# pansanity666/TransHuman

Measured on AMD Instinct MI355X. Metric: rays/sec (512x512, 64 samples/ray), higher is better.
Workload: dtype f32 (fp16 hi/lo x3 MFMA emulation)

## Files before the change

include/transhuman_hip.h:

```cpp
#ifndef TRANSHUMAN_HIP_H
#define TRANSHUMAN_HIP_H

#include <stddef.h>
#include <stdint.h>

#ifdef __cplusplus
extern "C" {
#endif

#define TH_ABI_VERSION 12

typedef struct th_ctx th_ctx;
typedef void* th_stream;

int         th_abi_version(void);
const char* th_last_error(void);
int         th_ctx_create(int device, th_ctx** out);
void        th_ctx_destroy(th_ctx* ctx);
size_t      th_sizeof(const char* type_name);

enum { TH_PROF_HULL = 0, TH_PROF_DPARF = 1, TH_PROF_GATHER = 2, TH_PROF_MLP = 3, TH_PROF_COMPOSITE = 4,
       TH_PROF_VIT = 5, TH_PROF_FOLD = 6 , TH_PROF_PHASES = 8 };
int th_profile_enable(th_ctx* ctx, int on);
int th_profile_read(th_ctx* ctx, double* ms_out, int64_t* count_out);
int th_host_wait_read(th_ctx* ctx, double* ms_out);
int th_clock_probe(th_ctx* ctx, int64_t* out_dev , th_stream stream);
int th_fused_cycles(th_ctx* ctx, int64_t* counters_dev);

typedef struct {
    const float* w;
    const float* b;
    int out_f;
    int in_f;
} th_linear;

typedef struct {
    th_linear fc_0, alpha_res_0;
    th_linear key0, val0;
    th_linear key1, val1;
    th_linear fc_1, fc_2, fc_3, alpha_fc;
    th_linear feature_fc, rgb_res_0, view_fc, rgb_res_1, fc_4, rgb_fc;
    th_linear upsample_color;
} th_mlp_weights;

typedef struct {
    const float *ln1_w, *ln1_b, *ln2_w, *ln2_b;
    th_linear qkv, proj, fc1, fc2;
} th_vit_block;

int th_set_mlp_weights(th_ctx* ctx, const th_mlp_weights* w, th_stream stream);
int th_set_mlp_mode(th_ctx* ctx, int mode);
int th_set_fused_waves(th_ctx* ctx, int waves);
int th_set_tok_gather(th_ctx* ctx, int on);
int th_set_tex_rows(th_ctx* ctx, int on);

#define TH_RANGE_SLOTS 8
#define TH_RANGE_FP16_LIMIT 0x7B53u
#define TH_RANGE_FP16_FLOOR 0x2400u
int th_set_vit_mode(th_ctx* ctx, int mode);
int th_range_snapshot(th_ctx* ctx, th_stream stream);
// ... 257 lines not shown
```

transhuman_amd/csrc/k_mlp_fused8_kernel.h:

```cpp
#pragma once
#include "k_mlp_fused_kernel.h"

typedef float f8_f4 __attribute__((ext_vector_type(4)));
typedef short f8_s4 __attribute__((ext_vector_type(4)));
typedef short f8_s8 __attribute__((ext_vector_type(8)));

#define F8_THREADS 512
#define F8_PART_FLOATS (3 * 8 * 32)
#define F8_PSTR 12
#define F8_MISC_FLOATS (F8_PSTR * 32 + F8_PART_FLOATS + 32 + 8)
#define F8_LDS_BYTES (ABUF_BYTES + MBUF_BYTES + F8_MISC_FLOATS * 4)
static_assert(F8_LDS_BYTES <= 163840, "the 8-wave tile must fit the CU's LDS");

#define F8_MFMA(A, B, C) __builtin_amdgcn_mfma_f32_16x16x32_f16((A), (B), (C), 0, 0, 0)

template <int CT>
__device__ __forceinline__ void f8_load_w(const uint4* __restrict__ wl, int t, uint4 (&w)[CT][2]) {
    const uint4* p = wl + (long long)t * (CT * 2 * 64);
#pragma unroll
    for (int c = 0; c < CT; ++c) {
        w[c][0] = p[(c * 2 + 0) * 64];
        w[c][1] = p[(c * 2 + 1) * 64];
    }
}
#define F8_WSLICE(L, wave, ct) ((L).w + (long long)(wave) * (L).KB * ((ct) * 2 * 64))

template <int NR, int ROWSTEP, bool PERM>
__device__ __forceinline__ void f8_load_x(const char* __restrict__ ahi, const char* __restrict__ alo, int aoff, int t,
                                          h8 (&xh)[NR], h8 (&xl)[NR]) {
    const int ko = (PERM ? 32 : 64) * t;
#pragma unroll
    for (int r = 0; r < NR; ++r) {
        xh[r] = *reinterpret_cast<const h8*>(ahi + r * ROWSTEP + aoff + ko);
        xl[r] = *reinterpret_cast<const h8*>(alo + r * ROWSTEP + aoff + ko);
    }
}
template <bool PERM>
__device__ __forceinline__ int f8_aoff(int lane, int str) {
    const int l = lane & 15, g = lane >> 4;
    return PERM ? l * str + 16 * (g >> 1) + 256 * (g & 1) : l * str + 16 * g;
}

template <int CT, int RT, int NR, int R0, bool FIRST>
__device__ __forceinline__ void f8_mfma_half(const uint4 (&w)[CT][2], const h8 (&xh)[NR], const h8 (&xl)[NR], f8_f4 (&acc)[CT][RT]) {
    const f8_f4 zero = {0.f, 0.f, 0.f, 0.f};
// ... 130 lines not shown
__device__ __forceinline__ void f8_mfma_dual(const uint4 (&r3)[2][2], const uint4 (&ra)[1][2], const h8 (&mh)[1], const h8 (&ml)[1],
                                             const h8 (&xh)[NV], const h8 (&xl)[NV], f8_f4 (&a3)[2][2], f8_f4 (&va)[1][RT]) {
    const f8_f4 zero = {0.f, 0.f, 0.f, 0.f};
#pragma unroll
    for (int t = 0; t < 3; ++t) {
        const int wp = t == 0 ? 1 : 0;
        const bool lo = t == 1;
        const bool first = FIRST && t == 0;
        a3[0][H] = F8_MFMA(*reinterpret_cast<const h8*>(&r3[0][wp]), lo ? ml[0] : mh[0], first ? zero : a3[0][H]);
#pragma unroll
        for (int r = 0; r < NV; ++r) {
            va[0][R0 + r] = F8_MFMA(*reinterpret_cast<const h8*>(&ra[0][wp]), lo ? xl[r] : xh[r], first ? zero : va[0][R0 + r]);
            if (r == 0) a3[1][H] = F8_MFMA(*reinterpret_cast<const h8*>(&r3[1][wp]), lo ? ml[0] : mh[0], first ? zero : a3[1][H]);
        }
    }
}

template <int V>
__global__ __launch_bounds__(F8_THREADS, 2) void mlp_fused8_kernel(FusedParams P_arg) {
#define PK P_arg
    struct F8Dbg { long long* dbg; };
    const F8Dbg P{PK.dbg};
    extern __shared__ __attribute__((aligned(16))) char lds[];
    char* abuf = lds;
    char* mbuf = lds + ABUF_BYTES;
    float* misc = reinterpret_cast<float*>(lds + ABUF_BYTES + MBUF_BYTES);
    float* probs = misc;
    float* part = misc + F8_PSTR * 32;
    float* sig = part + F8_PART_FLOATS;
    int* flag = reinterpret_cast<int*>(sig + 32);

    const int tid = threadIdx.x, lane = tid & 63, wave = tid >> 6;
    const int l15 = lane & 15, g4 = lane >> 4;
    const int tile = (int)((blockIdx.x & 7) * (gridDim.x >> 3) + (blockIdx.x >> 3));
    const int pbase = tile * FM_PTS;
    if (pbase >= PK.P) return;
    const int npts = min(FM_PTS, PK.P - pbase);
    const int fm_dbg_tile = tile;
    const int zoff = 0;
    constexpr int ROWS = 32 * V, RT = 2 * V;
    constexpr int RS256 = 16 * STR256;
    int dbg_i = 1;
    long long dbg_t = 0;
    long long* dbg_keep = reinterpret_cast<long long*>(flag + 2);
    constexpr float inv_v = 1.0f / (float)V;
    unsigned rmax = 0u;
    unsigned seen_s = 0u, seen_p = 0u, seen_n = 0u, seen_i = 0u, seen_4 = 0u;
    char* a256_lo = abuf + ROWS * STR256;

    struct TexPre { unsigned h0, h1; fm_u4 rq; };
    auto tex_fetch = [&]() __attribute__((always_inline)) {
        int tl = tile;
        asm volatile("" : "+s"(tl));
        TexPre t;
        const unsigned* hb = PK.tex_hdr + (long long)tl * 512;
        t.h0 = hb[lane];
        t.h1 = hb[64 + lane];
        t.rq = (fm_u4){0u, 0u, 0u, 0u};
        if (tid < 64 * V) t.rq = *reinterpret_cast<const fm_u4*>(PK.tex_rec + (long long)tl * V * 32 * 8 + tid * 4);
        return t;
    };
    auto fill_tex = [&](const TexPre& pre, auto rgb, auto&& under) __attribute__((always_inline)) {
        constexpr bool RGB = decltype(rgb)::value;
        constexpr int TSTR = 1040, TMAX = 103, NK = (TMAX + 7) / 8, NR = 4 * V;
        static_assert(TMAX * TSTR <= ABUF_BYTES, "a pass of texel rows must fit the operand buffer");
        int wv = __builtin_amdgcn_readfirstlane(wave), tl = tile;
        asm volatile("" : "+s"(wv), "+s"(tl));
        const unsigned* hb = PK.tex_hdr + (long long)tl * 512;
        unsigned h0 = pre.h0, h1 = pre.h1;
        const int npass = __builtin_amdgcn_readfirstlane((int)(h0 >> 16));
        char* recl = reinterpret_cast<char*>(misc);
        static_assert(32 * V * 32 <= (F8_PSTR * 32 + F8_PART_FLOATS) * 4, "row records must fit probs + part");
        unsigned fv[NR][4] = {};
        f32x2 bias_lo = {0.f, 0.f}, bias_hi = {0.f, 0.f};
        if constexpr (!RGB) {
            const float4 b4 = *reinterpret_cast<const float4*>(PK.ar0.bias + 4 * lane);
            bias_lo = (f32x2){b4.x, b4.y};
            bias_hi = (f32x2){b4.z, b4.w};
        }
        for (int p = 0; p < npass; ++p) {
            if (p > 0) {
                FM_SYNCL();
                h0 = hb[p * 128 + lane];
                h1 = hb[p * 128 + 64 + lane];
            }
            const int U = __builtin_amdgcn_readfirstlane((int)(h0 & 0xffffu));
            {
                constexpr int NA = 7, NB = 10;
                const char* mbase = reinterpret_cast<const char*>(RGB ? PK.tex_map2 : PK.tex_map);
                const unsigned loff = (unsigned)lane * 16u;
                const int last = U - 1;
                fm_u4 ta[NA], tb[NB - NA], tc[NK - NB];
#pragma unroll
                for (int k = 0; k < NA; ++k) {
                    const int i = min(wv + 8 * k, last);
                    const unsigned id = (unsigned)__builtin_amdgcn_readlane((int)h0, 8 + i);
                    ta[k] = *reinterpret_cast<const fm_u4*>(mbase + TX_ADDR(id));
                }
                const bool more = U > 8 * NA, most = U > 8 * NB;
                if (more) {
#pragma unroll
                    for (int k = NA; k < NB; ++k) {
                        const int i = min(wv + 8 * k, last);
                        const unsigned id = (unsigned)__builtin_amdgcn_readlane((int)h1, i - 56);
                        tb[k - NA] = *reinterpret_cast<const fm_u4*>(mbase + TX_ADDR(id));
                    }
                }
                if (most) {
#pragma unroll
                    for (int k = NB; k < NK; ++k) {
                        const int i = min(wv + 8 * k, last);
                        const unsigned id = (unsigned)__builtin_amdgcn_readlane((int)h1, i - 56);
                        tc[k - NB] = *reinterpret_cast<const fm_u4*>(mbase + TX_ADDR(id));
                    }
                }
                if (p == 0) {
                    under();
                    if (tid < 64 * V) *reinterpret_cast<fm_u4*>(recl + tid * 16) = pre.rq;
                }
                int wv2 = wv;
                asm volatile("" : "+s"(wv2));
#pragma unroll
                for (int k = 0; k < NA; ++k) *reinterpret_cast<fm_u4*>(abuf + min(wv2 + 8 * k, last) * TSTR + lane * 16) = ta[k];
                if (more) {
#pragma unroll
                    for (int k = NA; k < NB; ++k) *reinterpret_cast<fm_u4*>(abuf + min(wv2 + 8 * k, last) * TSTR + lane * 16) = tb[k - NA];
                }
                if (most) {
#pragma unroll
                    for (int k = NB; k < NK; ++k) *reinterpret_cast<fm_u4*>(abuf + min(wv2 + 8 * k, last) * TSTR + lane * 16) = tc[k - NB];
                }
            }
            FM_SYNCL();
            const int sh2 = npass == 1 ? 2 : npass == 2 ? 1 : 0;
            const int cofs = lane * 16;
            struct RowIn { float4 a, b, c, d; fm_u4 q0; };
            auto issue = [&](int k, const fm_u4& o, RowIn& r) __attribute__((always_inline)) {
                r.q0 = *reinterpret_cast<const fm_u4*>(recl + (wv + 8 * k) * 32);
                r.a = *reinterpret_cast<const float4*>(abuf + (o[0] + cofs));
                r.b = *reinterpret_cast<const float4*>(abuf + (o[1] + cofs));
                r.c = *reinterpret_cast<const float4*>(abuf + (o[2] + cofs));
                r.d = *reinterpret_cast<const float4*>(abuf + (o[3] + cofs));
            };
            auto offs = [&](int k) __attribute__((always_inline)) {
                return *reinterpret_cast<const fm_u4*>(recl + (wv + 8 * k) * 32 + 16);
            };
            auto blend = [&](int k, const RowIn& r, auto sel) __attribute__((always_inline)) {
// ... 15 lines not shown
                    n2 = __builtin_bit_cast(unsigned, h0f); n3 = __builtin_bit_cast(unsigned, h1f);
                } else {
                    lo = __builtin_elementwise_max(lo + bias_lo, (f32x2){0.f, 0.f});
                    hi = __builtin_elementwise_max(hi + bias_hi, (f32x2){0.f, 0.f});
                    split_pair(lo[0], lo[1], n0, n2);
                    split_pair(hi[0], hi[1], n1, n3);
                }
                if constexpr (decltype(sel)::value) {
                    const bool mine = ((k & 3) >> sh2) == p;
                    fv[k][0] = mine ? n0 : fv[k][0]; fv[k][1] = mine ? n1 : fv[k][1];
                    fv[k][2] = mine ? n2 : fv[k][2]; fv[k][3] = mine ? n3 : fv[k][3];
                } else {
                    fv[k][0] = n0; fv[k][1] = n1; fv[k][2] = n2; fv[k][3] = n3;
                }
            };
            auto rows_loop = [&](auto sel) __attribute__((always_inline)) {
                RowIn in[2];
                fm_u4 of[2];
                of[0] = offs(0);
                of[1] = offs(1);
                issue(0, of[0], in[0]);
#pragma unroll
                for (int k = 0; k < NR; ++k) {
                    if (k + 1 < NR) issue(k + 1, of[(k + 1) & 1], in[(k + 1) & 1]);
                    if (k + 2 < NR) of[k & 1] = offs(k + 2);
                    FM_SB();
                    blend(k, in[k & 1], sel);
                    FM_SB();
                }
            };
            if (npass == 1) rows_loop(std::false_type{});
            else rows_loop(std::true_type{});
        }
        FM_SYNCL();
        if constexpr (RGB) {
#pragma unroll
            for (int k = 0; k < NR; ++k)
                *reinterpret_cast<fm_u4*>(abuf + (wv + 8 * k) * TSTR + lane * 16) = (fm_u4){fv[k][0], fv[k][1], fv[k][2], fv[k][3]};
        } else {
#pragma unroll
            for (int k = 0; k < NR; ++k) {
                range_acc<true>(rmax, fv[k][0]);
                range_acc<true>(rmax, fv[k][1]);
                *reinterpret_cast<uint2*>(abuf + (wv + 8 * k) * STR256 + lane * 8) = make_uint2(fv[k][0], fv[k][1]);
                *reinterpret_cast<uint2*>(a256_lo + (wv + 8 * k) * STR256 + lane * 8) = make_uint2(fv[k][2], fv[k][3]);
            }
            range_commit(PK.range, TH_RANGE_P, seen_p, rmax);
        }
    };

    if (PK.dbg != nullptr && tid == 0 && (tile & 15) == 0) {
        atomicAdd(reinterpret_cast<unsigned long long*>(PK.dbg), 1ull);
        dbg_t = clock64();
        dbg_keep[0] = dbg_t;
        dbg_keep[1] = wall_clock64();
    }
    fm_u4 rv4 = {0u, 0u, 0u, 0u};
    unsigned rv1 = 0u;
    static_assert(TH_RANGE_S == 1 && TH_RANGE_P == 2 && TH_RANGE_N == 3 && TH_RANGE_INTER == 4 && TH_RANGE_F4 == 5, "range slots 1..5");
    if (PK.range != nullptr) {
        const unsigned* rtab = PK.range + zoff;
        rv4 = (fm_u4){rtab[1], rtab[2], rtab[3], rtab[4]};
        rv1 = rtab[5];
    }
    TexPre tex_pre = tex_fetch(), tex_pre2;

    int vsel[2] = {0, 0};
    float vdv[2] = {0.f, 0.f};
    f8_f4 acc2[2][RT];
    {
        constexpr int STOK_STR = 1040;
        static_assert(32 * V * STOK_STR <= ABUF_BYTES, "T' rows must fit the operand buffer");
        char* pe_hi = mbuf;
        char* pe_lo = mbuf + 32 * STR64;
        const int pt = tid & 255, prow = pt >> 3, pc = pt & 7, ppl = tid >> 8;
        const int psrc = min(prow, npts - 1);
        const uint4 pe_v = *reinterpret_cast<const uint4*>(PK.pe + (long long)(pbase + psrc) * 128 + 64 * ppl + 8 * pc);
        char* wsp_hi = mbuf + 16384;
        char* wsp_lo = wsp_hi + 32 * STRVD;
        const unsigned* hdr = reinterpret_cast<const unsigned*>(PK.stok) + (long long)((PK.P + 31) / 32 * 32) * 16 + (long long)tile * 128;
        const unsigned h0 = hdr[lane], h1 = hdr[64 + lane];
        const int ns = tid / 7, nk = tid - 7 * ns;
        int slot = -1;
        float nw = 0.f;
        if (tid < 224) {
            const unsigned* rec = reinterpret_cast<const unsigned*>(PK.stok) + (long long)(pbase + min(ns, npts - 1)) * 16;
            slot = (int)rec[nk];
            nw = __builtin_bit_cast(float, rec[8 + nk]);
        }
        const unsigned zq = 0u;
        const float inv_t = PK.t_inv[zoff];
        uint4 wq[2][2][2];
        const uint4* wl = F8_WSLICE(PK.w16.fc_0pe, wave, 2) + lane;
        f8_load_w<2>(wl, 0, wq[0]);
        f8_load_w<2>(wl, 1, wq[1]);
        const float4 b0[2] = {f8_bias(PK.fc_0pe.bias, wave * 32, lane), f8_bias(PK.fc_0pe.bias, wave * 32 + 16, lane)};
        if (tid < 2 * 32 * STRVD / 16) reinterpret_cast<uint4*>(wsp_hi)[tid] = make_uint4(zq, zq, zq, zq);
        *reinterpret_cast<uint4*>((ppl ? pe_lo : pe_hi) + prow * STR64 + 16 * pc) = pe_v;
        const int U = __builtin_amdgcn_readfirstlane((int)h0);
        FM_SB();
        auto slot_centre = [&](int u) {
            const int d = (2 + u) >> 1;
            const unsigned src = d < 64 ? (unsigned)__builtin_amdgcn_readlane((int)h0, d) : (unsigned)__builtin_amdgcn_readlane((int)h1, d - 64);
            return (int)((src >> (16 * ((2 + u) & 1))) & 0xffffu);
        };
#pragma unroll
        for (int c = 0; c < 2; ++c)
#pragma unroll
            for (int r = 0; r < RT; ++r) acc2[c][r] = (f8_f4){0.f, 0.f, 0.f, 0.f};
        f8_f4 a1[2][2] = {{{0.f, 0.f, 0.f, 0.f}, {0.f, 0.f, 0.f, 0.f}}, {{0.f, 0.f, 0.f, 0.f}, {0.f, 0.f, 0.f, 0.f}}};
        const int wv = __builtin_amdgcn_readfirstlane(wave);
        const int aoffw = f8_aoff<false>(lane, STRVD), aoffp = f8_aoff<false>(lane, STR64);
        for (int u0 = 0; u0 < U; u0 += 32) {
            const int nU = min(32, U - u0);
            if (u0 > 0) {
                FM_SYNCL();
                if (tid < 2 * 32 * STRVD / 16) reinterpret_cast<uint4*>(wsp_hi)[tid] = make_uint4(zq, zq, zq, zq);
            }
            for (int u = wv; u < nU; u += 8) {
                const int cu = slot_centre(u0 + u);
                const char* g = reinterpret_cast<const char*>(PK.tsplit) + (long long)cu * 1024 + lane * 16;
#pragma unroll
                for (int vw = 0; vw < V; ++vw)
                    __builtin_amdgcn_global_load_lds((fm_gptr)(g + (long long)vw * PK.t_nc * 1024),
                                                     (fm_lptr)(abuf + (vw * 32 + u) * STOK_STR), 16, 0, 0);
            }
            FM_SYNCL();
            if (slot >= u0 && slot < u0 + 32) {
                _Float16 hi, lo;
                split_h(nw, hi, lo);
                *reinterpret_cast<_Float16*>(wsp_hi + ns * STRVD + 2 * (slot - u0)) = hi;
                *reinterpret_cast<_Float16*>(wsp_lo + ns * STRVD + 2 * (slot - u0)) = lo;
            }
            if (u0 == 0) {
#pragma unroll
                for (int t = 0; t < 2; ++t) {
                    h8 xh[2], xl[2];
                    f8_load_x<2, 16 * STR64, false>(pe_hi, pe_lo, aoffp, t, xh, xl);
                    if (t == 0) f8_mfma_half<2, 2, 2, 0, true>(wq[0], xh, xl, a1);
                    else f8_mfma_half<2, 2, 2, 0, false>(wq[1], xh, xl, a1);
                }
            }
            FM_SYNC();
            {
                h8 xh[2], xl[2];
                f8_load_x<2, 16 * STRVD, false>(wsp_hi, wsp_lo, aoffw, 0, xh, xl);
                const int tq = l15 >> 2, tc = 8 * (l15 & 3);
                const int ro0 = min(8 * g4 + tq, nU - 1) * STOK_STR + tc, ro1 = min(8 * g4 + 4 + tq, nU - 1) * STOK_STR + tc;
                typedef __attribute__((address_space(3))) f8_s4* f8_lp;
#pragma unroll
                for (int r = 0; r < V; ++r)
#pragma unroll
                    for (int c = 0; c < 2; ++c) {
                        const char* rb = abuf + r * 32 * STOK_STR + 2 * (wave * 32 + c * 16);
                        const f8_s4 h0 = __builtin_amdgcn_ds_read_tr16_b64_v4i16((f8_lp)(rb + ro0));
                        const f8_s4 h1 = __builtin_amdgcn_ds_read_tr16_b64_v4i16((f8_lp)(rb + ro1));
                        const f8_s4 l0 = __builtin_amdgcn_ds_read_tr16_b64_v4i16((f8_lp)(rb + ro0 + 512));
// ... 186 lines not shown
    f8_gemm_rt<RT, 2, RS256, true, true>(abuf, a256_lo, STR256, F8_WSLICE(PK.w16.fc_2, wave, 2), 8, lane, acc2, wk2);
    const float4 bi[2] = {f8_bias(PK.fc_2.bias, wave * 32, lane), f8_bias(PK.fc_2.bias, wave * 32 + 16, lane)};
#pragma unroll
    for (int q = 0; q < 2; ++q) {
        const int i = tid + F8_THREADS * q, row = i >> 5, c = i & 31;
        float x = 0.f;
        if (PK.rgb_all != 2 && c < 27 && row < npts) {
            const long long vr = PK.vd_sel ? (long long)(vsel[q] / PK.vd_div) : (long long)(pbase + row);
            x = PK.vd[vr * 27 + c];
        }
        vdv[q] = x;
    }
    FM_SYNCL();
#pragma unroll
    for (int c = 0; c < 2; ++c) {
#pragma unroll
        for (int r = 0; r < RT; ++r) acc2[c][r] = f8_finish(acc2[c][r], bi[c], PK.fc_2.inv_scale, true);
#pragma unroll
        for (int h = 0; h < 2; ++h) {
            f8_f4 m = acc2[c][h];
#pragma unroll
            for (int r = 1; r < V; ++r) m = m + acc2[c][2 * r + h];
            m = m * (f8_f4){inv_v, inv_v, inv_v, inv_v};
            f8_store_h<STR256>(m, h * 16 + l15, wave * 32 + c * 16, mbuf, mbuf + 32 * STR256, lane, rmax);
        }
#pragma unroll
        for (int r = 0; r < RT; ++r) f8_store_h<STR256>(acc2[c][r], r * 16 + l15, wave * 32 + c * 16, abuf, a256_lo, lane, rmax);
    }
    range_commit(PK.range, TH_RANGE_INTER, seen_i, rmax);
    FM_SYNCL();

    char* vd_hi = mbuf + MBUF_VD_OFF;
    char* vd_lo = vd_hi + 32 * STRVD;
    tex_pre2 = tex_fetch();
    f8_f4 va[1][RT];
    {
        f8_f4 a3[2][2];
        const float4 aw[2] = {f8_bias(PK.alpha_w, wave * 32, lane), f8_bias(PK.alpha_w, wave * 32 + 16, lane)};
        const float4 b3[2] = {f8_bias(PK.fc_3.bias, wave * 32, lane), f8_bias(PK.fc_3.bias, wave * 32 + 16, lane)};
        if (PK.rgb_all != 2) {
            constexpr int T = 8;
            const uint4* w3l = F8_WSLICE(PK.w16.fc_3, wave, 2) + lane;
            const uint4* wal = F8_WSLICE(PK.w16.vfA, wave, 1) + lane;
            const int aoff = f8_aoff<true>(lane, STR256);
            const char* mhi = mbuf;
            const char* mlo = mbuf + 32 * STR256;
            uint4 r3[2][2][2], ra[2][1][2];
            h8 mah[1], mal[1], xah[V], xal[V], mbh[1], mbl[1], xbh[V], xbl[V];
            f8_load_w<2>(w3l, 0, r3[0]);
            f8_load_w<1>(wal, 0, ra[0]);
            f8_load_x<1, RS256, true>(mhi, mlo, aoff, 0, mah, mal);
            f8_load_x<V, RS256, true>(abuf, a256_lo, aoff, 0, xah, xal);
            FM_SB();
            auto step = [&](auto first, auto par, int t) __attribute__((always_inline)) {
                constexpr bool F = decltype(first)::value;
                constexpr int PB = decltype(par)::value;
                const int tn = t + 1 < T ? t + 1 : T - 1;
                f8_load_x<1, RS256, true>(mhi + RS256, mlo + RS256, aoff, t, mbh, mbl);
                f8_load_x<V, RS256, true>(abuf + V * RS256, a256_lo + V * RS256, aoff, t, xbh, xbl);
                f8_load_w<2>(w3l, tn, r3[PB ^ 1]);
                f8_load_w<1>(wal, tn, ra[PB ^ 1]);
                f8_mfma_dual<RT, V, 0, 0, F>(r3[PB], ra[PB], mah, mal, xah, xal, a3, va);
                f8_interleave<2 + 2 * V + 6, 3 * (2 + V)>();
                f8_load_x<1, RS256, true>(mhi, mlo, aoff, tn, mah, mal);
                f8_load_x<V, RS256, true>(abuf, a256_lo, aoff, tn, xah, xal);
                f8_mfma_dual<RT, V, 1, V, F>(r3[PB], ra[PB], mbh, mbl, xbh, xbl, a3, va);
                f8_interleave<2 + 2 * V, 3 * (2 + V)>();
// ... 157 lines not shown
```

transhuman_amd/csrc/k_mlp_fused_host.hip:

```cpp
#include <stdio.h>
#include <stdlib.h>
#include <string.h>

#include "k_mlp_fused_kernel.h"
#include "k_mlp_fused8_kernel.h"

__global__ void pack_fused_kernel(const float* __restrict__ W, int N, int K, int KB, int CT, const int* __restrict__ cols,
                                  float scale, uint4* __restrict__ out) {
    long long total = 4LL * KB * CT * 2 * 64;
    for (long long o = blockIdx.x * (long long)blockDim.x + threadIdx.x; o < total;
         o += (long long)gridDim.x * blockDim.x) {
        int lane = (int)(o & 63);
        long long q = o >> 6;
        int plane = (int)(q & 1); q >>= 1;
        int ct = (int)(q % CT); q /= CT;
        int kb = (int)(q % KB);
        int wave = (int)(q / KB);
        int col = cols[wave * CT + ct] + (lane & 31);
        int k0 = 16 * kb + 8 * (lane >> 5);
        h8 v;
#pragma unroll
        for (int j = 0; j < 8; ++j) {
            int k = k0 + j;
            float x = (col < N && k < K) ? W[(long long)col * K + k] * scale : 0.f;
// ... 314 lines not shown
    return 0;
}

int th_map_fold_launch(const FusedParams& base, const float* map_split, int V, int H, int W, const int32_t* box, float* fold,
                       unsigned int* range, hipStream_t s, const unsigned* demand) {
    TH_REQUIRE(base.compact_ready, "the map fold needs the colour-folded layers (th_mlp_weights.upsample_color)");
    TH_REQUIRE(V >= 1 && H >= 1 && W >= 1 && map_split && fold, "bad argument");
    MapFoldParams p;
    p.ar0 = base.ar0c; p.rst = base.rstc;
    p.lat = map_split; p.rgb = map_split + (size_t)V * H * W * 256;
    p.box = box; p.V = V; p.H = H; p.W = W;
    p.out0 = fold; p.out12 = fold + (size_t)V * H * W * 256;
    p.range = range;
    p.list = nullptr; p.count = nullptr;
    static unsigned long long attr_done = 0ull;
    if (th_lds_attr_needed(&attr_done)) {
        TH_HIP(hipFuncSetAttribute((const void*)map_fold_kernel<false>, hipFuncAttributeMaxDynamicSharedMemorySize, 2 * MF_TEX * STR272));
        TH_HIP(hipFuncSetAttribute((const void*)map_fold_kernel<true>, hipFuncAttributeMaxDynamicSharedMemorySize, 2 * MF_TEX * STR272));
    }
    if (demand != nullptr) {
        const size_t NW = (size_t)V * H * W / 32;
        p.count = demand + 2 * NW;
        p.list = reinterpret_cast<const int32_t*>(demand + 2 * NW + 16);
        hipLaunchKernelGGL(map_fold_kernel<true>, dim3(512), dim3(256), 2 * MF_TEX * STR272, s, p);
        TH_LAUNCH_CHECK();
        return 0;
    }
    const int tpr = (W + MF_TEX - 1) / MF_TEX;
    hipLaunchKernelGGL(map_fold_kernel<false>, dim3((unsigned)(V * H * tpr)), dim3(256), 2 * MF_TEX * STR272, s, p);
    TH_LAUNCH_CHECK();
    return 0;
}

int th_mlp_fused_forward(const FusedParams& base, const ThMlpPacked& heads, int V, int P, const float* stok,
                         const void* pe, const void* f, int f_ld, const float* vd, const int32_t* vd_sel, int vd_div, int rgb_all, float* raw_c,
                         unsigned int* range, hipStream_t s, const void* tsplit, const float* t_inv, int t_nc, const float* tex_map,
                         size_t tex_stride) {
    if (P <= 0) return 0;
    TH_REQUIRE(V >= 1 && V <= 3, "fused MLP supports 1..3 reference views");
    TH_REQUIRE(f_ld == 384 || (f_ld == 272 && base.compact_ready),
               "pixel-feature rows must be 384 wide, or 272 wide with upsample_color weights uploaded");
    const bool cf = f_ld == 272;
    FusedParams p = base;
    if (cf) { p.ar0 = base.ar0c; p.rst = base.rstc; }
    p.alpha_w = heads.alpha_w; p.alpha_b = heads.alpha_b; p.rgb_w = heads.rgb_w; p.rgb_b = heads.rgb_b;
    TH_REQUIRE(tsplit == nullptr || (t_inv != nullptr && t_nc >= 7 && t_nc <= 4096), "split token table: scale word and 7 <= N_c <= 4096");
    p.tsplit = (const _Float16*)tsplit; p.t_inv = t_inv; p.t_nc = t_nc;
    const bool tex = tex_map != nullptr;
    TH_REQUIRE(!tex || (cf && f != nullptr), "texel hand-over: compact (272-wide) operand planes only");
    p.tex_hdr = nullptr; p.tex_rec = nullptr; p.tex_map = nullptr; p.tex_map2 = nullptr;
    if (tex) {
        p.tex_hdr = (const unsigned*)f;
        p.tex_rec = p.tex_hdr + (size_t)th_cdiv(P, FM_PTS) * 512;
        p.tex_map = tex_map;
        p.tex_map2 = tex_map + tex_stride;
        f = nullptr;
    }
    p.stok = stok; p.pe = (const _Float16*)pe; p.f = (const _Float16*)f; p.vd = vd; p.vd_sel = vd_sel; p.vd_div = vd_div > 0 ? vd_div : 1; p.raw_c = raw_c; p.P = P; p.rgb_all = rgb_all; p.range = range;
    static unsigned long long attr_done = 0ull;
    if (th_lds_attr_needed(&attr_done)) {
#define FM_ATTR(V_, F_)                                                                                       \
    TH_HIP(hipFuncSetAttribute((const void*)mlp_fused_kernel<V_, F_>, hipFuncAttributeMaxDynamicSharedMemorySize, \
                               FUSED_LDS_BYTES))
        FM_ATTR(1, 0); FM_ATTR(2, 0); FM_ATTR(3, 0); FM_ATTR(1, 1); FM_ATTR(2, 1); FM_ATTR(3, 1);
#undef FM_ATTR
#define FM_ATTR_T(V_)                                                                                              \
// ... 71 lines not shown
```

transhuman_amd/csrc/k_mlp_fused_kernel.h:

```cpp
#pragma once
#include <hip/hip_fp16.h>

#include <utility>

#include "th_internal.h"

typedef float f32x16 __attribute__((ext_vector_type(16)));
typedef _Float16 h8 __attribute__((ext_vector_type(8)));
typedef _Float16 h4 __attribute__((ext_vector_type(4)));
typedef float f32x4v __attribute__((ext_vector_type(4)));
typedef unsigned fm_u4 __attribute__((ext_vector_type(4)));

#define FM_PTS 32
#define STR272 560
#define STR256 528
#define STR192 400
#define STR128 272
#define STR64 144
#define STRVD 80
#define KSTR 132

#define ABUF_BYTES (2 * 96 * STR272)
#define MBUF_BYTES (96 * KSTR * 4)
#define MISC_FLOATS (9 * 32 + 128 + 4 * 32 * 4 + 8)
#define FUSED_LDS_BYTES (ABUF_BYTES + MBUF_BYTES + MISC_FLOATS * 4)
#define MBUF_VD_OFF 0
#define MBUF_FC4_OFF 8192

#define FM_SYNC_(BARRIER)                                                                                 \
    do {                                                                                                 \
        BARRIER;                                                                                         \
        if (FM_DBG_SAMPLED) {                                                                            \
            long long now_ = clock64();                                                                  \
            atomicAdd(reinterpret_cast<unsigned long long*>(P.dbg + dbg_i++), (unsigned long long)(now_ - dbg_t)); \
            dbg_t = now_;                                                                                \
        }                                                                                                \
    } while (0)
#define FM_DBG_SAMPLED (P.dbg != nullptr && tid == 0 && (fm_dbg_tile & 15) == 0)
#define FM_SYNC() FM_SYNC_(__syncthreads())
#define FM_LDS_BARRIER()                                                      \
    do {                                                                      \
        __builtin_amdgcn_fence(__ATOMIC_RELEASE, "workgroup", "local");       \
        __builtin_amdgcn_s_barrier();                                         \
        __builtin_amdgcn_fence(__ATOMIC_ACQUIRE, "workgroup", "local");       \
    } while (0)
#define FM_SYNCL() FM_SYNC_(FM_LDS_BARRIER())

#define FM_STAMP()                                                                                       \
    do {                                                                                                 \
        if (FM_DBG_SAMPLED) {                                                                            \
            long long now_ = clock64();                                                                  \
            atomicAdd(reinterpret_cast<unsigned long long*>(P.dbg + dbg_i++), (unsigned long long)(now_ - dbg_t)); \
            dbg_t = now_;                                                                                \
        }                                                                                                \
    } while (0)

__device__ __forceinline__ void split_h(float x, _Float16& hi, _Float16& lo) {
    hi = (_Float16)x;
    lo = (_Float16)(x - (float)hi);
}
typedef _Float16 h2v __attribute__((ext_vector_type(2)));
typedef float f32x2 __attribute__((ext_vector_type(2)));
__device__ __forceinline__ void split_pair(float x0, float x1, unsigned& hi, unsigned& lo) {
    h2v h;
    h[0] = (_Float16)x0;
    h[1] = (_Float16)x1;
    hi = *reinterpret_cast<unsigned*>(&h);
    asm("" : "+v"(hi));
    unsigned l;
    asm("v_fma_mixlo_f16 %0, %1, -1.0, %2 op_sel:[0,0,0] op_sel_hi:[1,0,0]" : "=v"(l) : "v"(hi), "v"(x0));
    asm("v_fma_mixhi_f16 %0, %1, -1.0, %2 op_sel:[1,0,0] op_sel_hi:[1,0,0]" : "+v"(l) : "v"(hi), "v"(x1));
    lo = l;
}

typedef __attribute__((address_space(1))) const void* fm_gptr;
typedef __attribute__((address_space(3))) void* fm_lptr;

template <int V, int KROW, int KC, int STR>
__device__ __forceinline__ void stage_glds(const _Float16* __restrict__ src, int coff, int pbase, int npts,
                                           char* __restrict__ hi, char* __restrict__ lo, int wave, int lane) {
    constexpr int SL = STR / 16, DS = (2 * KC) / 16, NS = 32 * V * SL;
    constexpr int NCH = (NS + 63) / 64;
    constexpr int DR = 256 / SL, DSL = 256 % SL;
    static_assert(STR % 16 == 0 && (2 * KC) % 16 == 0 && DS < SL, "row stride must hold the data slots plus a pad slot");
    const int wv = __builtin_amdgcn_readfirstlane(wave);
// ... 1317 lines not shown
```

transhuman_amd/csrc/th_internal.h:

```cpp
#pragma once
#include <hip/hip_runtime.h>
#include <stdint.h>
#include <stddef.h>
#include <time.h>
#include <string>

#include "transhuman_hip.h"

#define TH_WAVE 64

void th_set_error(const std::string& msg);
#define TH_FAIL(msg)                                                                \
    do {                                                                            \
        th_set_error(std::string(__func__) + ": " + (msg));                         \
        return -1;                                                                  \
    } while (0)
#define TH_REQUIRE(cond, msg)                                                       \
    do {                                                                            \
        if (!(cond)) TH_FAIL(msg);                                                  \
    } while (0)
#define TH_HIP(call)                                                                \
    do {                                                                            \
        hipError_t e__ = (call);                                                    \
        if (e__ != hipSuccess) {                                                    \
// ... 159 lines not shown
#endif

struct ThMlpPacked {
    ThPacked fc_0, alpha_res_0, kv0, kv1, fc_1, fc_2, fc_3, feature_fc, rgb_res_0, view_fc, rgb_res_1, fc_4;
    ThPacked fc_0tok;
    ThPacked alpha_res_0c, rgb_res_0c, rgb_res_1c;
    bool compact_ready = false;
    float *alpha_w = nullptr, *alpha_b = nullptr;
    float *rgb_w = nullptr, *rgb_b = nullptr;
    bool ready = false;
};
struct ThVitBlockPacked {
    float *ln1_w, *ln1_b, *ln2_w, *ln2_b;
    ThPacked qkv, proj, fc1, fc2;
};
struct ThVitPacked {
    int depth = 0, dim = 0, heads = 0;
    ThVitBlockPacked* blocks = nullptr;
    float *norm_w = nullptr, *norm_b = nullptr;
    bool ready = false;
};

struct FusedLayer {
    const uint4* w;
    const float* bias;
    float inv_scale;
    int CT, KB;
    float inv_scale2;
};
struct Fused16 {
    FusedLayer fc_0pe, kv1, kv0, fc_2, fc_3, fc_4, vfA, vfD;
};
struct FusedParams {
    Fused16 w16;
    int waves;
    FusedLayer fc_0pe;
    FusedLayer kv1, ar0, kv0, fc_1, fc_2, fc_3, fc_4;
    FusedLayer vfA, vfD, rst;
    FusedLayer ar0c, rstc;
    bool compact_ready;
    const float *alpha_w, *alpha_b, *rgb_w, *rgb_b;
    const float* stok;
    const _Float16* tsplit;
    const float* t_inv;
    int t_nc;
    const _Float16* pe;
    const _Float16* f;
    const unsigned* tex_hdr;
    const unsigned* tex_rec;
    const float* tex_map;
    const float* tex_map2;
    const float* vd;
    const int32_t* vd_sel;
    int vd_div;
    float* raw_c;
    int P;
    int rgb_all;
    unsigned int* range;
    long long* dbg;
    long long* cycles_buf;
};
enum { TH_RANGE_F = 0, TH_RANGE_S = 1, TH_RANGE_P = 2, TH_RANGE_N = 3, TH_RANGE_INTER = 4, TH_RANGE_F4 = 5, TH_RANGE_CONV = 6,
       TH_RANGE_VIT = 7 };
size_t th_fused_pack_bytes();
int th_fused_pack(const th_mlp_weights* w, const th_linear* folded, void* store, FusedParams* out, hipStream_t s);
int th_mlp_fused_forward(const FusedParams& base, const ThMlpPacked& heads, int V, int P, const float* stok,
                         const void* pe, const void* f, int f_ld, const float* vd, const int32_t* vd_sel, int vd_div, int rgb_all,
                         float* raw_c, unsigned int* range, hipStream_t s, const void* tsplit = nullptr,
                         const float* t_inv = nullptr, int t_nc = 0, const float* tex_map = nullptr, size_t tex_stride = 0);
static inline bool th_lds_attr_needed(unsigned long long* done) {
    int dev = 0;
    if (hipGetDevice(&dev) != hipSuccess || dev < 0 || dev > 63) return true;
    if ((*done >> dev) & 1ull) return false;
    *done |= 1ull << dev;
    return true;
}
int th_map_fold_launch(const FusedParams& base, const float* map_split, int V, int H, int W, const int32_t* box, float* fold,
                       unsigned int* range, hipStream_t s, const unsigned* demand = nullptr );
size_t th_pixtex_bytes(int V, long long P);
int th_pixtex_launch(int V, int H, int W, const ThPointSrc* ps, const int32_t* sel, int P, const float* cams,
                     const float* scale, void* out, hipStream_t s);
int th_tok_split(float* tprime, int rows, float* sc, unsigned int* range, hipStream_t s);

struct th_ctx {
    void* fused_store = nullptr;
    FusedParams fused{};
    bool fused_ready = false;
    int mlp_mode = 1;
    int vit_mode = 1;
    int tok_gather = 1;
    int tex_rows = 1;
    int device = 0;
// ... 168 lines not shown
```

transhuman_amd/hip.py:

```python
import ctypes as C
import os

import torch

_HERE = os.path.dirname(os.path.abspath(__file__))
LIB_PATH = os.environ.get("TH_LIB_PATH") or os.path.join(_HERE, "libtranshuman_hip.so")

c_float_p = C.POINTER(C.c_float)


class ThLinear(C.Structure):
    _fields_ = [("w", C.c_void_p), ("b", C.c_void_p), ("out_f", C.c_int), ("in_f", C.c_int)]


class ThMlpWeights(C.Structure):
    _names = ["fc_0", "alpha_res_0", "key0", "val0", "key1", "val1", "fc_1", "fc_2", "fc_3", "alpha_fc",
              "feature_fc", "rgb_res_0", "view_fc", "rgb_res_1", "fc_4", "rgb_fc", "upsample_color"]
    _fields_ = [(n, ThLinear) for n in _names]


class ThSmplModel(C.Structure):
    _fields_ = [("v_template", C.c_void_p), ("shapedirs", C.c_void_p), ("posedirs", C.c_void_p),
                ("J_regressor", C.c_void_p), ("weights", C.c_void_p), ("parent", C.c_void_p), ("n_verts", C.c_int)]

# ... 1 lines not shown
class ThVitBlock(C.Structure):
    _fields_ = [("ln1_w", C.c_void_p), ("ln1_b", C.c_void_p), ("ln2_w", C.c_void_p), ("ln2_b", C.c_void_p),
                ("qkv", ThLinear), ("proj", ThLinear), ("fc1", ThLinear), ("fc2", ThLinear)]


class ThPoints(C.Structure):
    _fields_ = [("pts", C.c_void_p), ("ray_o", C.c_void_p), ("ray_d", C.c_void_p), ("near", C.c_void_p),
                ("far", C.c_void_p), ("t_vals", C.c_void_p), ("one_minus_t", C.c_void_p), ("R", C.c_int),
                ("S", C.c_int), ("z_vals", C.c_void_p), ("sigma_noise", C.c_void_p)]


class ThFrame(C.Structure):
    _fields_ = [("verts_world", C.c_void_p), ("n_verts", C.c_int), ("Rh", C.c_void_p), ("Th", C.c_void_p),
                ("cams", C.c_void_p), ("scale_xy", C.c_void_p), ("pixel_map_nhwc", C.c_void_p), ("V", C.c_int),
                ("H", C.c_int), ("W", C.c_int), ("map_channels", C.c_int), ("tokens", C.c_void_p), ("centres", C.c_void_p),
                ("rot", C.c_void_p), ("n_clusters", C.c_int), ("hull_thresh", C.c_float),
                ("small_frame_rays", C.c_int), ("map_source", C.c_void_p), ("map_fold", C.c_void_p)]


class ThMapSource(C.Structure):
    _fields_ = [("box", C.c_void_p), ("reach", C.c_float), ("img", C.c_void_p), ("lat0", C.c_void_p),
                ("lat1", C.c_void_p), ("lat2", C.c_void_p), ("dims", C.c_int32 * 6), ("demand", C.c_void_p)]


SYMBOLS = {
    "th_abi_version": (C.c_int, []),
    "th_last_error": (C.c_char_p, []),
    "th_sizeof": (C.c_size_t, [C.c_char_p]),
    "th_ctx_create": (C.c_int, [C.c_int, C.POINTER(C.c_void_p)]),
    "th_ctx_destroy": (None, [C.c_void_p]),
    "th_profile_enable": (C.c_int, [C.c_void_p, C.c_int]),
    "th_profile_read": (C.c_int, [C.c_void_p, C.POINTER(C.c_double), C.POINTER(C.c_int64)]),
    "th_fused_cycles": (C.c_int, [C.c_void_p, C.c_void_p]),
    "th_host_wait_read": (C.c_int, [C.c_void_p, C.POINTER(C.c_double)]),
    "th_clock_probe": (C.c_int, [C.c_void_p, C.c_void_p, C.c_void_p]),
    "th_set_mlp_weights": (C.c_int, [C.c_void_p, C.POINTER(ThMlpWeights), C.c_void_p]),
    "th_set_mlp_mode": (C.c_int, [C.c_void_p, C.c_int]),
    "th_set_fused_waves": (C.c_int, [C.c_void_p, C.c_int]),
    "th_set_vit_mode": (C.c_int, [C.c_void_p, C.c_int]),
    "th_set_tok_gather": (C.c_int, [C.c_void_p, C.c_int]),
    "th_set_tex_rows": (C.c_int, [C.c_void_p, C.c_int]),
    "th_map_fold": (C.c_int, [C.c_void_p, C.c_void_p, C.c_int, C.c_int, C.c_int, C.c_void_p, C.c_void_p, C.c_void_p]),
    "th_pixel_texlist_bytes": (C.c_size_t, [C.c_int, C.c_int]),
    "th_pixel_texlist": (C.c_int, [C.c_void_p, C.c_void_p, C.c_int, C.c_int, C.c_int, C.c_void_p, C.c_void_p, C.c_int,
                                   C.c_void_p, C.c_void_p, C.c_void_p, C.c_size_t, C.c_void_p]),
    "th_range_snapshot": (C.c_int, [C.c_void_p, C.c_void_p]),
    "th_range_read": (C.c_int, [C.c_void_p, C.c_int, C.POINTER(C.c_uint32)]),
    "th_range_last_slot": (C.c_int, [C.c_void_p]),
    "th_set_chunk_samples": (C.c_int, [C.c_int]),
    "th_set_vit_weights": (C.c_int, [C.c_void_p, C.c_int, C.c_int, C.c_int, C.POINTER(ThVitBlock), C.c_void_p,
                                     C.c_void_p, C.c_void_p]),
    "th_linear_workspace_bytes": (C.c_size_t, [C.c_int, C.c_int]),
    "th_linear_forward": (C.c_int, [C.c_void_p, C.c_void_p, C.c_int, C.c_int, C.POINTER(ThLinear), C.c_int,
                                    C.c_void_p, C.c_int, C.c_void_p, C.c_size_t, C.c_void_p]),
    "th_hull_workspace_bytes": (C.c_size_t, [C.c_int]),
    "th_hull_mask": (C.c_int, [C.c_void_p, C.POINTER(ThPoints), C.c_void_p, C.c_int, C.c_float, C.c_void_p,
                               C.c_void_p, C.c_void_p, C.c_size_t, C.c_void_p]),
    "th_paint_group": (C.c_int, [C.c_void_p, C.c_void_p, C.c_int, C.c_int, C.c_int, C.c_int, C.c_void_p, C.c_int,
                                 C.c_void_p, C.c_void_p, C.c_void_p, C.c_void_p, C.c_void_p, C.c_int, C.c_void_p,
                                 C.c_void_p, C.c_void_p]),
    "th_segment_mean_f32": (C.c_int, [C.c_void_p, C.c_void_p, C.c_int, C.c_void_p, C.c_void_p, C.c_int, C.c_void_p,
                                      C.c_void_p]),
    "th_segment_mean_rot_f64": (C.c_int, [C.c_void_p, C.c_void_p, C.c_void_p, C.c_void_p, C.c_int, C.c_void_p,
                                          C.c_void_p]),
    "th_upsample_concat_nhwc": (C.c_int, [C.c_void_p, C.c_void_p, C.c_void_p, C.c_void_p, C.c_void_p,
                                          C.POINTER(C.c_int32), C.c_int, C.c_int, C.c_int, C.c_void_p, C.c_void_p,
# ... 1415 lines not shown
```

Baseline: 17.75 million.

## Prefetch a later tile's inputs during texture fill and front-load kernel argument loads

During the RGB texture fill pass, each thread issues one dummy load that touches a tile F8_WARM_D positions ahead in the same XCD slice. The load covers that tile's neighbour headers and records, positional encodings and texture headers and records, so they are warm in cache when that tile's block starts. The kernel prologue is also reordered: hot kernel arguments are moved to the front of FusedParams and read early, and inline asm forces the remaining scalar argument loads before the early return. The range table and record loads become unconditional, using clamped addresses, and out-of-range blocks now return only after these loads. In exchange the change adds extra global traffic, scalar register pressure and some wasted work in surplus blocks, and it adds a host helper for inspecting the warm-tile mapping.

```diff
diff --git a/include/transhuman_hip.h b/include/transhuman_hip.h
--- a/include/transhuman_hip.h
+++ b/include/transhuman_hip.h
@@ -26,6 +26,7 @@
 int th_host_wait_read(th_ctx* ctx, double* ms_out);
 int th_clock_probe(th_ctx* ctx, int64_t* out_dev , th_stream stream);
 int th_fused_cycles(th_ctx* ctx, int64_t* counters_dev);
+int th_fused_warm_tile(int tile, int ntiles, int* distance_out);
 
 typedef struct {
     const float* w;
diff --git a/transhuman_amd/csrc/k_mlp_fused8_kernel.h b/transhuman_amd/csrc/k_mlp_fused8_kernel.h
--- a/transhuman_amd/csrc/k_mlp_fused8_kernel.h
+++ b/transhuman_amd/csrc/k_mlp_fused8_kernel.h
@@ -11,6 +11,17 @@
 #define F8_MISC_FLOATS (F8_PSTR * 32 + F8_PART_FLOATS + 32 + 8)
 #define F8_LDS_BYTES (ABUF_BYTES + MBUF_BYTES + F8_MISC_FLOATS * 4)
 static_assert(F8_LDS_BYTES <= 163840, "the 8-wave tile must fit the CU's LDS");
+
+#ifndef F8_WARM_D
+#define F8_WARM_D 32
+#endif
+__host__ __device__ __forceinline__ int f8_warm_tile(int tile, int ntiles) {
+    const int per_xcd = (ntiles + 7) >> 3;
+    const int lo = tile / per_xcd * per_xcd;
+    const int hi = lo + per_xcd < ntiles ? lo + per_xcd : ntiles;
+    if (hi - lo < F8_WARM_D) return tile;
+    return tile + F8_WARM_D < hi ? tile + F8_WARM_D : hi - 1;
+}
 
 #define F8_MFMA(A, B, C) __builtin_amdgcn_mfma_f32_16x16x32_f16((A), (B), (C), 0, 0, 0)
 
@@ -207,10 +218,21 @@
 
     const int tid = threadIdx.x, lane = tid & 63, wave = tid >> 6;
     const int l15 = lane & 15, g4 = lane >> 4;
-    const int tile = (int)((blockIdx.x & 7) * (gridDim.x >> 3) + (blockIdx.x >> 3));
+    const int a_P = PK.P, a_tnc = PK.t_nc, a_kb0 = PK.w16.fc_0pe.KB;
+    const float* a_stok = PK.stok;
+    const _Float16* a_pe = PK.pe;
+    const unsigned* a_thdr = PK.tex_hdr;
+    const unsigned* a_trec = PK.tex_rec;
+    const unsigned* a_range = PK.range;
+    const _Float16* a_tsplit = PK.tsplit;
+    const float* a_tinv = PK.t_inv;
+    const long long* a_dbg = PK.dbg;
+    const uint4* a_w0 = PK.w16.fc_0pe.w;
+    const float* a_b0 = PK.w16.fc_0pe.bias;
+    const int tile_raw = (int)((blockIdx.x & 7) * (gridDim.x >> 3) + (blockIdx.x >> 3));
+    const int tile = min(tile_raw, (a_P - 1) / FM_PTS);
     const int pbase = tile * FM_PTS;
-    if (pbase >= PK.P) return;
-    const int npts = min(FM_PTS, PK.P - pbase);
+    const int npts = min(FM_PTS, a_P - pbase);
     const int fm_dbg_tile = tile;
     const int zoff = 0;
     constexpr int ROWS = 32 * V, RT = 2 * V;
@@ -224,15 +246,14 @@
     char* a256_lo = abuf + ROWS * STR256;
 
     struct TexPre { unsigned h0, h1; fm_u4 rq; };
-    auto tex_fetch = [&]() __attribute__((always_inline)) {
+    auto tex_fetch = [&](const unsigned* thdr, const unsigned* trec) __attribute__((always_inline)) {
         int tl = tile;
         asm volatile("" : "+s"(tl));
         TexPre t;
-        const unsigned* hb = PK.tex_hdr + (long long)tl * 512;
+        const unsigned* hb = thdr + (long long)tl * 512;
         t.h0 = hb[lane];
         t.h1 = hb[64 + lane];
-        t.rq = (fm_u4){0u, 0u, 0u, 0u};
-        if (tid < 64 * V) t.rq = *reinterpret_cast<const fm_u4*>(PK.tex_rec + (long long)tl * V * 32 * 8 + tid * 4);
+        t.rq = *reinterpret_cast<const fm_u4*>(trec + (long long)tl * V * 32 * 8 + min(tid, 64 * V - 1) * 4);
         return t;
     };
     auto fill_tex = [&](const TexPre& pre, auto rgb, auto&& under) __attribute__((always_inline)) {
@@ -247,6 +268,7 @@
         char* recl = reinterpret_cast<char*>(misc);
         static_assert(32 * V * 32 <= (F8_PSTR * 32 + F8_PART_FLOATS) * 4, "row records must fit probs + part");
         unsigned fv[NR][4] = {};
+        unsigned warm = 0u;
         f32x2 bias_lo = {0.f, 0.f}, bias_hi = {0.f, 0.f};
         if constexpr (!RGB) {
             const float4 b4 = *reinterpret_cast<const float4*>(PK.ar0.bias + 4 * lane);
@@ -288,6 +310,20 @@
                         const unsigned id = (unsigned)__builtin_amdgcn_readlane((int)h1, i - 56);
                         tc[k - NB] = *reinterpret_cast<const fm_u4*>(mbase + TX_ADDR(id));
                     }
+                }
+                if constexpr (RGB) {
+                    const int wi = wave * 16 + (lane >> 2);
+                    const int tw = f8_warm_tile(tile, (PK.P + FM_PTS - 1) / FM_PTS);
+                    const char* w_nbr = reinterpret_cast<const char*>(PK.stok);
+                    const long long o_hdr = ((long long)((PK.P + 31) / 32 * 32) * 16 + (long long)tw * 128) * 4 + wi * 128;
+                    const long long o_rec = (long long)tw * FM_PTS * 64 + (wi - 4) * 128;
+                    const long long o_pe = min((long long)tw * FM_PTS * 256 + (wi - 20) * 128, (long long)PK.P * 256 - 128);
+                    const long long o_th = (long long)tw * 2048 + (wi - 84) * 128;
+                    const long long o_tr = (long long)tw * V * 1024 + min(wi - 88, 8 * V - 1) * 128;
+                    const char* wp = wi < 20 ? w_nbr : wi < 84 ? reinterpret_cast<const char*>(PK.pe)
+                                   : wi < 88 ? reinterpret_cast<const char*>(PK.tex_hdr) : reinterpret_cast<const char*>(PK.tex_rec);
+                    const long long wo = wi < 4 ? o_hdr : wi < 20 ? o_rec : wi < 84 ? o_pe : wi < 88 ? o_th : o_tr;
+                    warm = *reinterpret_cast<const unsigned*>(wp + wo);
                 }
                 if (p == 0) {
                     under();
@@ -369,6 +405,7 @@
             if (npass == 1) rows_loop(std::false_type{});
             else rows_loop(std::true_type{});
         }
+        if constexpr (RGB) asm volatile("" : : "v"(warm));
         FM_SYNCL();
         if constexpr (RGB) {
 #pragma unroll
@@ -386,21 +423,16 @@
         }
     };
 
-    if (PK.dbg != nullptr && tid == 0 && (tile & 15) == 0) {
-        atomicAdd(reinterpret_cast<unsigned long long*>(PK.dbg), 1ull);
-        dbg_t = clock64();
-        dbg_keep[0] = dbg_t;
-        dbg_keep[1] = wall_clock64();
-    }
+    const long long dbg_start = clock64();
     fm_u4 rv4 = {0u, 0u, 0u, 0u};
     unsigned rv1 = 0u;
     static_assert(TH_RANGE_S == 1 && TH_RANGE_P == 2 && TH_RANGE_N == 3 && TH_RANGE_INTER == 4 && TH_RANGE_F4 == 5, "range slots 1..5");
-    if (PK.range != nullptr) {
-        const unsigned* rtab = PK.range + zoff;
+    {
+        const unsigned* rtab = a_range != nullptr ? a_range + zoff : reinterpret_cast<const unsigned*>(a_stok);
         rv4 = (fm_u4){rtab[1], rtab[2], rtab[3], rtab[4]};
         rv1 = rtab[5];
     }
-    TexPre tex_pre = tex_fetch(), tex_pre2;
+    TexPre tex_pre = tex_fetch(a_thdr, a_trec), tex_pre2;
 
     int vsel[2] = {0, 0};
     float vdv[2] = {0.f, 0.f};
@@ -412,26 +444,39 @@
         char* pe_lo = mbuf + 32 * STR64;
         const int pt = tid & 255, prow = pt >> 3, pc = pt & 7, ppl = tid >> 8;
         const int psrc = min(prow, npts - 1);
-        const uint4 pe_v = *reinterpret_cast<const uint4*>(PK.pe + (long long)(pbase + psrc) * 128 + 64 * ppl + 8 * pc);
+        const uint4 pe_v = *reinterpret_cast<const uint4*>(a_pe + (long long)(pbase + psrc) * 128 + 64 * ppl + 8 * pc);
         char* wsp_hi = mbuf + 16384;
         char* wsp_lo = wsp_hi + 32 * STRVD;
-        const unsigned* hdr = reinterpret_cast<const unsigned*>(PK.stok) + (long long)((PK.P + 31) / 32 * 32) * 16 + (long long)tile * 128;
+        const unsigned* hdr = reinterpret_cast<const unsigned*>(a_stok) + (long long)((a_P + 31) / 32 * 32) * 16 + (long long)tile * 128;
         const unsigned h0 = hdr[lane], h1 = hdr[64 + lane];
         const int ns = tid / 7, nk = tid - 7 * ns;
-        int slot = -1;
-        float nw = 0.f;
-        if (tid < 224) {
-            const unsigned* rec = reinterpret_cast<const unsigned*>(PK.stok) + (long long)(pbase + min(ns, npts - 1)) * 16;
-            slot = (int)rec[nk];
-            nw = __builtin_bit_cast(float, rec[8 + nk]);
-        }
+        const unsigned* rec = reinterpret_cast<const unsigned*>(a_stok) + (long long)(pbase + min(ns, npts - 1)) * 16;
+        const unsigned rec_s = rec[nk], rec_w = rec[8 + nk];
+        const int slot = tid < 224 ? (int)rec_s : -1;
+        const float nw = tid < 224 ? __builtin_bit_cast(float, rec_w) : 0.f;
         const unsigned zq = 0u;
-        const float inv_t = PK.t_inv[zoff];
+        const float inv_t = a_tinv[zoff];
         uint4 wq[2][2][2];
-        const uint4* wl = F8_WSLICE(PK.w16.fc_0pe, wave, 2) + lane;
+        const uint4* wl = a_w0 + (long long)wave * a_kb0 * (2 * 2 * 64) + lane;
         f8_load_w<2>(wl, 0, wq[0]);
         f8_load_w<2>(wl, 1, wq[1]);
-        const float4 b0[2] = {f8_bias(PK.fc_0pe.bias, wave * 32, lane), f8_bias(PK.fc_0pe.bias, wave * 32 + 16, lane)};
+        const float4 b0[2] = {f8_bias(a_b0, wave * 32, lane), f8_bias(a_b0, wave * 32 + 16, lane)};
+        asm volatile("" : : "s"(PK.w16.kv1.w), "s"(PK.w16.kv1.KB), "s"(PK.w16.kv0.w), "s"(PK.w16.kv0.KB), "s"(PK.w16.fc_2.w),
+                     "s"(PK.w16.fc_2.KB), "s"(PK.w16.fc_3.w), "s"(PK.w16.fc_3.KB), "s"(PK.w16.vfA.w), "s"(PK.w16.vfA.KB),
+                     "s"(PK.w16.vfD.w), "s"(PK.w16.vfD.KB), "s"(PK.w16.fc_4.w), "s"(PK.w16.fc_4.KB), "s"(PK.fc_0pe.inv_scale),
+                     "s"(PK.kv1.bias), "s"(PK.kv1.inv_scale), "s"(PK.ar0.bias), "s"(PK.kv0.bias), "s"(PK.kv0.inv_scale),
+                     "s"(PK.fc_1.bias), "s"(PK.fc_2.bias), "s"(PK.fc_2.inv_scale), "s"(PK.fc_3.bias), "s"(PK.fc_3.inv_scale));
+        asm volatile("" : : "s"(PK.fc_4.bias), "s"(PK.fc_4.inv_scale), "s"(PK.rst.bias), "s"(PK.rst.inv_scale), "s"(PK.alpha_w),
+                     "s"(PK.alpha_b), "s"(PK.rgb_w), "s"(PK.rgb_b), "s"(PK.tex_map), "s"(PK.tex_map2), "s"(PK.vd), "s"(PK.vd_sel),
+                     "s"(PK.vd_div), "s"(PK.raw_c), "s"(PK.rgb_all));
+        asm volatile("" ::: "memory");
+        if (tile_raw != tile) return;
+        if (a_dbg != nullptr && tid == 0 && (tile & 15) == 0) {
+            atomicAdd(reinterpret_cast<unsigned long long*>(PK.dbg), 1ull);
+            dbg_t = dbg_start;
+            dbg_keep[0] = dbg_t;
+            dbg_keep[1] = wall_clock64();
+        }
         if (tid < 2 * 32 * STRVD / 16) reinterpret_cast<uint4*>(wsp_hi)[tid] = make_uint4(zq, zq, zq, zq);
         *reinterpret_cast<uint4*>((ppl ? pe_lo : pe_hi) + prow * STR64 + 16 * pc) = pe_v;
         const int U = __builtin_amdgcn_readfirstlane((int)h0);
@@ -456,10 +501,10 @@
             }
             for (int u = wv; u < nU; u += 8) {
                 const int cu = slot_centre(u0 + u);
-                const char* g = reinterpret_cast<const char*>(PK.tsplit) + (long long)cu * 1024 + lane * 16;
+                const char* g = reinterpret_cast<const char*>(a_tsplit) + (long long)cu * 1024 + lane * 16;
 #pragma unroll
                 for (int vw = 0; vw < V; ++vw)
-                    __builtin_amdgcn_global_load_lds((fm_gptr)(g + (long long)vw * PK.t_nc * 1024),
+                    __builtin_amdgcn_global_load_lds((fm_gptr)(g + (long long)vw * a_tnc * 1024),
                                                      (fm_lptr)(abuf + (vw * 32 + u) * STOK_STR), 16, 0, 0);
             }
             FM_SYNCL();
@@ -712,7 +757,7 @@
 
     char* vd_hi = mbuf + MBUF_VD_OFF;
     char* vd_lo = vd_hi + 32 * STRVD;
-    tex_pre2 = tex_fetch();
+    tex_pre2 = tex_fetch(PK.tex_hdr, PK.tex_rec);
     f8_f4 va[1][RT];
     {
         f8_f4 a3[2][2];
diff --git a/transhuman_amd/csrc/k_mlp_fused_host.hip b/transhuman_amd/csrc/k_mlp_fused_host.hip
--- a/transhuman_amd/csrc/k_mlp_fused_host.hip
+++ b/transhuman_amd/csrc/k_mlp_fused_host.hip
@@ -370,6 +370,12 @@
     return 0;
 }
 
+extern "C" int th_fused_warm_tile(int tile, int ntiles, int* distance_out) {
+    if (distance_out != nullptr) *distance_out = F8_WARM_D;
+    if (ntiles < 1 || tile < 0 || tile >= ntiles) return -1;
+    return f8_warm_tile(tile, ntiles);
+}
+
 int th_mlp_fused_forward(const FusedParams& base, const ThMlpPacked& heads, int V, int P, const float* stok,
                          const void* pe, const void* f, int f_ld, const float* vd, const int32_t* vd_sel, int vd_div, int rgb_all, float* raw_c,
                          unsigned int* range, hipStream_t s, const void* tsplit, const float* t_inv, int t_nc, const float* tex_map,
diff --git a/transhuman_amd/csrc/k_mlp_fused_kernel.h b/transhuman_amd/csrc/k_mlp_fused_kernel.h
--- a/transhuman_amd/csrc/k_mlp_fused_kernel.h
+++ b/transhuman_amd/csrc/k_mlp_fused_kernel.h
@@ -27,12 +27,14 @@
 #define MBUF_VD_OFF 0
 #define MBUF_FC4_OFF 8192
 
+#define FM_DBG_LAST 61
 #define FM_SYNC_(BARRIER)                                                                                 \
     do {                                                                                                 \
         BARRIER;                                                                                         \
         if (FM_DBG_SAMPLED) {                                                                            \
             long long now_ = clock64();                                                                  \
-            atomicAdd(reinterpret_cast<unsigned long long*>(P.dbg + dbg_i++), (unsigned long long)(now_ - dbg_t)); \
+            atomicAdd(reinterpret_cast<unsigned long long*>(P.dbg + dbg_i), (unsigned long long)(now_ - dbg_t)); \
+            dbg_i = dbg_i < FM_DBG_LAST ? dbg_i + 1 : FM_DBG_LAST;                                       \
             dbg_t = now_;                                                                                \
         }                                                                                                \
     } while (0)
@@ -50,7 +52,8 @@
     do {                                                                                                 \
         if (FM_DBG_SAMPLED) {                                                                            \
             long long now_ = clock64();                                                                  \
-            atomicAdd(reinterpret_cast<unsigned long long*>(P.dbg + dbg_i++), (unsigned long long)(now_ - dbg_t)); \
+            atomicAdd(reinterpret_cast<unsigned long long*>(P.dbg + dbg_i), (unsigned long long)(now_ - dbg_t)); \
+            dbg_i = dbg_i < FM_DBG_LAST ? dbg_i + 1 : FM_DBG_LAST;                                       \
             dbg_t = now_;                                                                                \
         }                                                                                                \
     } while (0)
diff --git a/transhuman_amd/csrc/th_internal.h b/transhuman_amd/csrc/th_internal.h
--- a/transhuman_amd/csrc/th_internal.h
+++ b/transhuman_amd/csrc/th_internal.h
@@ -215,6 +215,16 @@
     FusedLayer fc_0pe, kv1, kv0, fc_2, fc_3, fc_4, vfA, vfD;
 };
 struct FusedParams {
+    int P;
+    int t_nc;
+    const float* stok;
+    const _Float16* pe;
+    const unsigned* tex_hdr;
+    const unsigned* tex_rec;
+    unsigned int* range;
+    const _Float16* tsplit;
+    const float* t_inv;
+    long long* dbg;
     Fused16 w16;
     int waves;
     FusedLayer fc_0pe;
@@ -223,24 +233,14 @@
     FusedLayer ar0c, rstc;
     bool compact_ready;
     const float *alpha_w, *alpha_b, *rgb_w, *rgb_b;
-    const float* stok;
-    const _Float16* tsplit;
-    const float* t_inv;
-    int t_nc;
-    const _Float16* pe;
     const _Float16* f;
-    const unsigned* tex_hdr;
-    const unsigned* tex_rec;
     const float* tex_map;
     const float* tex_map2;
     const float* vd;
     const int32_t* vd_sel;
     int vd_div;
     float* raw_c;
-    int P;
     int rgb_all;
-    unsigned int* range;
-    long long* dbg;
     long long* cycles_buf;
 };
 enum { TH_RANGE_F = 0, TH_RANGE_S = 1, TH_RANGE_P = 2, TH_RANGE_N = 3, TH_RANGE_INTER = 4, TH_RANGE_F4 = 5, TH_RANGE_CONV = 6,
diff --git a/transhuman_amd/hip.py b/transhuman_amd/hip.py
--- a/transhuman_amd/hip.py
+++ b/transhuman_amd/hip.py
@@ -57,6 +57,7 @@
     "th_profile_enable": (C.c_int, [C.c_void_p, C.c_int]),
     "th_profile_read": (C.c_int, [C.c_void_p, C.POINTER(C.c_double), C.POINTER(C.c_int64)]),
     "th_fused_cycles": (C.c_int, [C.c_void_p, C.c_void_p]),
+    "th_fused_warm_tile": (C.c_int, [C.c_int, C.c_int, C.POINTER(C.c_int)]),
     "th_host_wait_read": (C.c_int, [C.c_void_p, C.POINTER(C.c_double)]),
     "th_clock_probe": (C.c_int, [C.c_void_p, C.c_void_p, C.c_void_p]),
     "th_set_mlp_weights": (C.c_int, [C.c_void_p, C.POINTER(ThMlpWeights), C.c_void_p]),
```

New measurement: 17.69 million. About the same (-0.3%).
